# dmalyuta/explicit_hybrid_mpc

Hardware: AMD Instinct MI355X
Metric: oracle LP solves/sec + final regions/sec, 4-state 2-input N=5 hybrid MPC (higher is better)
Workload: dtype f64

## Files before the change

explicit_hybrid_mpc_amd/build.py:

```python

import os
import shutil
import subprocess
from concurrent.futures import ThreadPoolExecutor

HERE = os.path.dirname(os.path.abspath(__file__))
SRC_DIR = os.path.join(HERE, 'csrc')
LIB_DIR = os.path.join(HERE, 'lib')
OBJ_DIR = os.path.join(LIB_DIR, 'obj')
LIB = os.path.join(LIB_DIR, 'libehmpc.so')
def _headers():
    hs = sorted(f for f in os.listdir(SRC_DIR) if f.endswith('.h'))
    return hs + [os.path.join('..', '..', 'include', 'ehmpc.h')]


HEADERS = _headers()
K2_NPS = (8, 12, 16, 20, 24, 28, 32)
K2_SLOTS = (1, 2, 3, 4)
K2Q_NPS = (8, 16, 24, 32)
KP_INSTANCES = tuple((d, e, sl) for (d, e) in ((12, 8), (16, 8), (16, 12), (20, 12), (20, 16),
                                                (24, 16), (24, 20), (28, 20), (28, 24), (32, 24),
                                                (32, 28)) for sl in (2, 3)) + \
    ((16, 12, 4), (28, 20, 4), (32, 24, 4))
KPM_INSTANCES = KP_INSTANCES
K3_RS = (2, 4)
MIDFIRST = '-DEHM_PERSIST_MIDFIRST=1'
FLAGS = ['--offload-arch=gfx950', '-O3', '-std=c++17', '-fPIC', '-Wno-unused-result',
         '-fvisibility=hidden', '-fvisibility-inlines-hidden']
FLAGS += os.environ.get('EHM_BUILD_FLAGS', '').split()
_TAG = os.environ.get('EHM_BUILD_TAG', '')
if _TAG:
    OBJ_DIR = os.path.join(LIB_DIR, 'obj_' + _TAG)
    LIB = os.path.join(LIB_DIR, 'libehmpc_%s.so' % _TAG)


def _hipcc():
    for cand in (os.environ.get('HIPCC'), shutil.which('hipcc'), '/opt/rocm/bin/hipcc'):
        if cand and os.path.exists(cand):
            return cand
    raise RuntimeError('hipcc not found: libehmpc.so cannot be built')


def _cxx():
    for cand in (os.environ.get('CXX'), shutil.which('g++'), shutil.which('c++')):
        if cand and os.path.exists(cand):
            return cand
    return _hipcc()


_INC_CACHE = {}


def _includes(path):
    path = os.path.normpath(path)
    if path in _INC_CACHE:
        return _INC_CACHE[path]
    _INC_CACHE[path] = found = set()
    try:
        text = open(path).read()
    except OSError:
        return found
    import re
    for inc in re.findall(r'^\s*#\s*include\s+"([^"]+)"', text, flags=re.M):
        dep = os.path.normpath(os.path.join(os.path.dirname(path), inc))
        if os.path.exists(dep):
            found.add(dep)
            found |= _includes(dep)
    return found


def _dep_mtime(src=None):
    if src is None:
        deps = [os.path.normpath(os.path.join(SRC_DIR, h)) for h in HEADERS]
    else:
        deps = list(_includes(src))
    deps += [__file__]
    return max(os.path.getmtime(d) for d in deps)


SEARCH_SRC = os.path.join(SRC_DIR, 'ehm_search.cpp')
SEARCH_OBJ = os.path.join(OBJ_DIR, 'ehm_search.o')
FRONTIER_SRC = os.path.join(SRC_DIR, 'ehm_frontier.cpp')
FRONTIER_OBJ = os.path.join(OBJ_DIR, 'ehm_frontier.o')
SEARCH_DEPS = [SEARCH_SRC, os.path.normpath(os.path.join(HERE, '..', 'include', 'ehm_search.h')),
               os.path.normpath(os.path.join(HERE, '..', 'include', 'ehmpc.h'))]
FRONTIER_DEPS = [FRONTIER_SRC,
                 os.path.normpath(os.path.join(HERE, '..', 'include', 'ehm_frontier.h'))] + \
    SEARCH_DEPS[1:]
HOST_OBJECTS = ((SEARCH_OBJ, SEARCH_SRC, SEARCH_DEPS), (FRONTIER_OBJ, FRONTIER_SRC, FRONTIER_DEPS))


def _objects():
    objs = [(os.path.join(OBJ_DIR, 'ehm_capi.o'), os.path.join(SRC_DIR, 'ehm_capi.hip'), []),
            (os.path.join(OBJ_DIR, 'ehm_explicit.o'), os.path.join(SRC_DIR, 'ehm_explicit.hip'),
             []),
            (os.path.join(OBJ_DIR, 'ehm_implicit.o'), os.path.join(SRC_DIR, 'ehm_implicit.hip'),
             [])]
    for np_ in K2_NPS:
        for sl in K2_SLOTS:
            objs.append((os.path.join(OBJ_DIR, 'ehm_k2_%d_%d.o' % (np_, sl)),
                         os.path.join(SRC_DIR, 'ehm_k2.hip'),
                         ['-DEHM_NP=%d' % np_, '-DEHM_SLOTS=%d' % sl, MIDFIRST]))
    for np_ in K2Q_NPS:
        for sl in K2_SLOTS:
            objs.append((os.path.join(OBJ_DIR, 'ehm_k2q_%d_%d.o' % (np_, sl)),
                         os.path.join(SRC_DIR, 'ehm_k2.hip'),
                         ['-DEHM_NP=%d' % np_, '-DEHM_SLOTS=%d' % sl, '-DEHM2_QUAD=1', MIDFIRST]))
    for npd, npe, sl in KP_INSTANCES:
        objs.append((os.path.join(OBJ_DIR, 'ehm_kp_%d_%d_%d.o' % (npd, npe, sl)),
                     os.path.join(SRC_DIR, 'ehm_kp.hip'),
                     ['-DEHM_NPD=%d' % npd, '-DEHM_NPE=%d' % npe, '-DEHM_SLOTS=%d' % sl]))
    for npd, npe, sl in KPM_INSTANCES:
        objs.append((os.path.join(OBJ_DIR, 'ehm_kpm_%d_%d_%d.o' % (npd, npe, sl)),
                     os.path.join(SRC_DIR, 'ehm_kp.hip'),
                     ['-DEHM_NPD=%d' % npd, '-DEHM_NPE=%d' % npe, '-DEHM_SLOTS=%d' % sl,
                      '-DEHM_PERSIST_MIDFIRST=1']))
    for rs in K3_RS:
        objs.append((os.path.join(OBJ_DIR, 'ehm_k3_%d.o' % rs),
                     os.path.join(SRC_DIR, 'ehm_k3.hip'),
                     ['-DEHM3_RS=%d' % rs, '-mllvm', '-pragma-unroll-threshold=200000']))
    objs.append((os.path.join(OBJ_DIR, 'ehm_k4.o'), os.path.join(SRC_DIR, 'ehm_k4.hip'), []))
    return objs


def _stale(obj, src, dep_t):
    return (not os.path.exists(obj) or
            os.path.getmtime(obj) < max(dep_t, os.path.getmtime(src)))


def is_stale():
    if not os.path.exists(LIB):
        return True
    t = os.path.getmtime(LIB)
    srcs = [os.path.join(SRC_DIR, f)
            for f in ('ehm_capi.hip', 'ehm_k2.hip', 'ehm_k3.hip', 'ehm_k4.hip', 'ehm_kp.hip',
                      'ehm_explicit.hip', 'ehm_implicit.hip')]
    return max([_dep_mtime()] + [os.path.getmtime(s)
                                 for s in srcs + SEARCH_DEPS + FRONTIER_DEPS]) > t


def build(force=False, verbose=False, jobs=None):
    if not force and not is_stale():
        return LIB
    os.makedirs(OBJ_DIR, exist_ok=True)
    hipcc = _hipcc()
    todo = [(o, s, f) for (o, s, f) in _objects() if force or _stale(o, s, _dep_mtime(s))]

    def compile_one(item):
        obj, src, extra = item
        cmd = [hipcc] + FLAGS + extra + ['-c', src, '-o', obj]
        if verbose:
            print(' '.join(cmd))
        subprocess.check_call(cmd)

    jobs = jobs or max(1, (os.cpu_count() or 2))
    with ThreadPoolExecutor(max_workers=jobs) as pool:
        list(pool.map(compile_one, todo))
    for obj, src, deps in HOST_OBJECTS:
        if force or not os.path.exists(obj) or \
                os.path.getmtime(obj) < max(os.path.getmtime(d) for d in deps):
            cmd = [_cxx(), '-O2', '-std=c++17', '-fPIC', '-Wall', '-fvisibility=hidden', '-fvisibility-inlines-hidden',
                   '-c', src, '-o', obj]
            if verbose:
                print(' '.join(cmd))
            subprocess.check_call(cmd)
    cmd = [hipcc, '--offload-arch=gfx950', '-shared', '-fPIC'] + [o for (o, _, _) in _objects()]
    cmd += [obj for obj, _, _ in HOST_OBJECTS]
    cmd += ['-o', LIB]
    if verbose:
        print(' '.join(cmd))
    subprocess.check_call(cmd)
    return LIB


if __name__ == '__main__':
    print(build(force=True, verbose=True))
```

explicit_hybrid_mpc_amd/csrc/ehm_ipm2.h:

```cpp
#include "ehm_dev.h"

#ifndef EHM_NP
#error "EHM_NP (column capacity, multiple of 4) must be defined"
#endif
#ifndef EHM_SLOTS
#error "EHM_SLOTS (row slots per lane) must be defined"
#endif

#ifndef EHM2_UNROLL
#define EHM2_UNROLL 2
#endif
#ifndef EHM2_FORM_MFMA
#define EHM2_FORM_MFMA 0
#endif
#ifndef EHM2_LU_CHUNK
#define EHM2_LU_CHUNK 8
#endif
#define EHM2_TOL_RES      1e-10
#define EHM2_TOL_GAP      1e-10
#define EHM2_MAX_ITER     40
#define EHM2_STEP_FRAC    0.999
#define EHM2_STEP_FRAC_SAFE 0.99
#define EHM2_STEP_FRAC_LAST 0.9
#define EHM2_ATTEMPTS     3
#define EHM2_PIVOT_REL    1e-13
#define EHM2_PIVOT_BIG    1e128
#define EHM2_STALL_ZONE   1e4
#define EHM2_ACCEPT_MERIT 1e3

#define EHM2_CAT2(a, b, c) a##b##_##c
#define EHM2_CAT(a, b, c) EHM2_CAT2(a, b, c)
#ifndef EHM2_QUAD
#define EHM2_QUAD 0
#endif
#if EHM2_QUAD
#define EHM2_NS EHM2_CAT(ehm2q_, EHM_NP, EHM_SLOTS)
#else
#define EHM2_NS EHM2_CAT(ehm2_, EHM_NP, EHM_SLOTS)
#endif

#ifndef EHM2_PROF
#define EHM2_PROF 0
#endif

namespace EHM2_NS {

using namespace ehm;

#if EHM2_PROF
#define EHM2_PT(k)                                                                   \
    {                                                                                \
        const long long _t = (long long)__builtin_readcyclecounter();               \
        if (lane0 == 0) W.pf[k] += (unsigned long long)(_t - _tp);                   \
        _tp = _t;                                                                    \
    }
#define EHM2_PDUMP()                                                                 \
    {                                                                                \
        wsync();                                                                     \
        if (S.gprof && lane0 < 24)                                                   \
            atomicAdd(&S.gprof[lane0], W.pf[lane0] + (lane0 == 23 ? 1ULL : 0ULL));   \
    }
#elif defined(EHM2_ISA_MARKS)
#define EHM2_PT(k) asm volatile("; @@PHASE " #k);
#define EHM2_PDUMP()
#else
#define EHM2_PT(k)
#define EHM2_PDUMP()
#endif

constexpr int NP = EHM_NP;
constexpr int SLOTS = EHM_SLOTS;
constexpr int MROWS = 64 * SLOTS;

__device__ __forceinline__ void wsync() {
    __builtin_amdgcn_fence(__ATOMIC_ACQ_REL, "wavefront");
    __builtin_amdgcn_wave_barrier();
}

template <int CTRL, int ROW_MASK>
__device__ __forceinline__ double dpp_move(double identity, double v) {
    const int lo = __builtin_amdgcn_update_dpp(__double2loint(identity), __double2loint(v), CTRL,
                                               ROW_MASK, 0xf, false);
    const int hi = __builtin_amdgcn_update_dpp(__double2hiint(identity), __double2hiint(v), CTRL,
                                               ROW_MASK, 0xf, false);
    return __hiloint2double(hi, lo);
}
__device__ __forceinline__ double lane63(double v) {
    const int lo = __builtin_amdgcn_readlane(__double2loint(v), 63);
    const int hi = __builtin_amdgcn_readlane(__double2hiint(v), 63);
    return __hiloint2double(hi, lo);
}
#define EHM2_DPP_REDUCE(OP, IDENT)                                       \
    v = OP(v, dpp_move<0x111, 0xf>(IDENT, v));                           \
    v = OP(v, dpp_move<0x112, 0xf>(IDENT, v));                           \
    v = OP(v, dpp_move<0x114, 0xf>(IDENT, v));                           \
    v = OP(v, dpp_move<0x118, 0xf>(IDENT, v));                           \
    v = OP(v, dpp_move<0x142, 0xa>(IDENT, v));                           \
    v = OP(v, dpp_move<0x143, 0xc>(IDENT, v));                           \
    return lane63(v);
__device__ __forceinline__ double op_add(double a, double b) { return a + b; }
__device__ __forceinline__ double op_max(double a, double b) { return fmax(a, b); }
__device__ __forceinline__ double op_min(double a, double b) { return fmin(a, b); }
#ifdef EHM2_REDUCE_SHFL
__device__ __forceinline__ double wave_sum(double v) {
    for (int o = 32; o > 0; o >>= 1) v += __shfl_xor(v, o, 64);
    return v;
}
__device__ __forceinline__ double wave_max(double v) {
    for (int o = 32; o > 0; o >>= 1) v = fmax(v, __shfl_xor(v, o, 64));
    return v;
}
#else
__device__ __forceinline__ double wave_sum(double v) { EHM2_DPP_REDUCE(op_add, 0.0) }
__device__ __forceinline__ double wave_max(double v) {
    EHM2_DPP_REDUCE(op_max, -__builtin_huge_val())
}
#endif
__device__ __forceinline__ double readlane_d(double v, int src) {
    const int lo = __builtin_amdgcn_readlane(__double2loint(v), src);
    const int hi = __builtin_amdgcn_readlane(__double2hiint(v), src);
    return __hiloint2double(hi, lo);
}
__device__ __forceinline__ int pin(int x) {
    asm volatile("" : "+v"(x));
    return x;
}
typedef __attribute__((address_space(3))) const volatile double lds_cvdouble;
__device__ __forceinline__ double lds1(const double* p) {
    return *(lds_cvdouble*)p;
}
__device__ __forceinline__ double uniform_d(double v) {
    int lo, hi;
    asm("s_nop 0\n\tv_readfirstlane_b32 %0, %2\n\tv_readfirstlane_b32 %1, %3\n\ts_nop 1"
        : "=s"(lo), "=s"(hi)
        : "v"(__double2loint(v)), "v"(__double2hiint(v)));
    return __hiloint2double(hi, lo);
}
__device__ __forceinline__ double const_d(double literal) {
    int lo = __double2loint(literal), hi = __double2hiint(literal);
    asm volatile("" : "+s"(lo), "+s"(hi));
    return __hiloint2double(hi, lo);
}
__device__ __forceinline__ double frcp(double x) {
    double r = __builtin_amdgcn_rcp(x);
    double e = fma(-x, r, 1.0);
    r = fma(r, e, r);
    e = fma(-x, r, 1.0);
    r = fma(r, e, r);
    return r;
}

struct Shared {
    const double* Wc;
    const double* wv;
    const double* cv;
    const double* aE;
    const double* eval;
    const int* erow;
    const int* eidx;
    int n, m, p, lda;
    int nd0, nE, LE;
    int colS, colOne, colZero;
#if EHM2_PROF
    unsigned long long* gprof;
#endif
};
__host__ __device__ inline size_t shared_doubles(const DevProblem& P) {
    return (((size_t)P.tot4 + (P.wc_lds ? P.m + P.n : 0)) + 1) & ~(size_t)1;
}
__device__ inline void carve_shared(Shared& S, double* base, const DevProblem& P) {
    S.n = P.n; S.m = P.m; S.p = P.p; S.lda = P.lda4;
    S.nd0 = P.nd0; S.nE = P.n - P.nd0; S.LE = P.LE4;
    S.colS = P.nd0; S.colOne = P.nd0 + P.p; S.colZero = P.nd0 + P.p + 1;
#if EHM2_PROF
    S.gprof = nullptr;
#endif
    S.Wc = base;
    S.aE = base + (size_t)(P.nd0 + P.p + 2) * P.lda4;
    S.eval = base + (size_t)P.ncw4 * P.lda4;
    S.erow = reinterpret_cast<const int*>(S.eval + (size_t)S.nE * S.LE);
    S.eidx = S.erow + (size_t)S.nE * S.LE;
    if (P.wc_lds) {
        S.wv = base + P.tot4;
        S.cv = S.wv + P.m;
    } else {
        S.wv = P.w;
        S.cv = P.c;
    }
}
__device__ inline void use_commutation(Shared& S, const DevProblem& P, int d) {
    if (!P.wc_lds) S.wv = P.w + (size_t)d * P.m;
}
__device__ inline void load_shared(const DevProblem& P, int d, double* base, int tid, int nthr) {
    const int tot = P.tot4;
    const double* src = P.Wc4 + (size_t)d * tot;
    for (int k = tid; k < tot; k += nthr) base[k] = src[k];
    if (P.wc_lds) {
        const double* wd = P.w + (size_t)d * P.m;
        for (int k = tid; k < P.m; k += nthr) base[tot + k] = wd[k];
        for (int k = tid; k < P.n; k += nthr) base[tot + P.m + k] = P.c[k];
    }
}

struct Wave {
    double* M;
    double* X;
    double* vm0;
    double* vm1;
    double* c;
    double* x;
    double* xb;
    double* t;
    double* ub;
    double* db;
    double* sc;
    int n_lp, ne, ldx, ldm, xbase;
    int nr;
    int nE;
    int n_lin;
    int spec_col;
    int n_mpc;
    const double* E;
    double* yv;
    int psi0, npsi;
    int nsx;
    double sign_floor;
    double* gE;
    double* iD;
    double* qE;
    double* hX;
    double* xh;
    double* dn;
#if EHM2_PROF
    unsigned long long* pf;
#endif
#if EHM2_QUAD
    double* Q;
    double* qv;
    double* a1;
    double* a2;
    double* gv;
    double* lq;
    int quad;
    int eq;
    double kap0, kap1, kap2, v0, bq1, bq2;
#endif
};
constexpr int LDM = NP + 1;
constexpr int GS = NP + 1;
typedef double double2v __attribute__((ext_vector_type(2)));
typedef double double4v __attribute__((ext_vector_type(4)));

__host__ __device__ constexpr int u_row_start(int k) {
    return (k & 1) ? (k * NP - 2 * (k / 2) * (k / 2)) : (k * NP - 2 * (k / 2) * (k / 2 - 1));
}
__host__ __device__ constexpr int uoff(int k) { return u_row_start(k) - (k & ~1); }
constexpr int U_SIZE = NP * (NP + 2) / 2;
constexpr size_t A_MIN = (size_t)U_SIZE + 256 + MROWS;
constexpr size_t A_KS = 512;
constexpr size_t A_SQ = ((size_t)NP * LDM < A_KS) ? A_KS : (size_t)NP * LDM;
constexpr size_t A_DOUBLES = (A_MIN < A_SQ) ? A_SQ : A_MIN;
__host__ __device__ inline int dense_rows(int ne, int p) { return (ne > p) ? ne - (p + 1) : ne; }
__host__ __device__ inline size_t wave_lp_doubles(int n_lp, int ne, int nE, int p) {
    const int kd = dense_rows(ne, p);
    const size_t ldx = kd ? ((size_t)kd | 1) : 0;
    const size_t nf = ((size_t)n_lp + 1) & ~(size_t)1;
    const size_t nEp = ((size_t)nE + 1) & ~(size_t)1;
    size_t tot = A_DOUBLES + (size_t)n_lp * ldx + 4 * nf + 2 * (size_t)NP + ((size_t)NP + 16) +
                 (size_t)nE * GS + 4 * nEp + 2 * (size_t)NP + 8;
#if EHM2_QUAD
    tot += 5 * (size_t)NP + (size_t)NP * LDM + 2;
#endif
#if EHM2_PROF
    tot += 24;
#endif
    return (tot + 1) & ~(size_t)1;
}
__device__ inline void carve_wave(Wave& W, double* base, int n_lp, int ne, int m, int nE, int nsx) {
    W.n_lp = n_lp;
    W.nE = nE;
    W.nr = n_lp - nE;
    W.ne = ne;
    W.ldm = LDM;
    W.ldx = (ne > nsx) ? ((ne - nsx) | 1) : 0;
    W.xbase = lp_xbase(m, ne);
    if (ne > 0 && W.xbase < 64 * (SLOTS - 1)) W.xbase = 64 * (SLOTS - 1);
    const int nf = (n_lp + 1) & ~1;
    const int nEp = (nE + 1) & ~1;
    W.M = base;
    W.vm0 = base + U_SIZE;
    W.sc = base + U_SIZE;
    W.vm1 = base + U_SIZE + 256;
    base += A_DOUBLES;
    W.X = base;   base += (size_t)n_lp * W.ldx;
    W.c = base;   base += nf;
    W.x = base;   base += nf;
    W.xb = base;  base += nf;
    W.t = base;   base += nf;
    W.ub = base;  base += NP;
    W.db = base;  base += NP;
    W.yv = base;  base += NP + 16;
    W.gE = base;  base += (size_t)nE * GS;
    W.iD = base;  base += nEp;
    W.qE = base;  base += nEp;
    W.hX = base;  base += 2 * nEp;
    W.xh = base;  base += 2 * NP;
    W.dn = base;  base += 8;
#if EHM2_PROF
    W.pf = reinterpret_cast<unsigned long long*>(base);  base += 24;
#endif
#if EHM2_QUAD
    W.qv = base;  base += NP;
    W.a1 = base;  base += NP;
    W.a2 = base;  base += NP;
    W.gv = base;  base += NP;
    W.lq = base;  base += 2;
    W.Q = base;
    W.quad = 0;
    W.eq = -1;
// ... 380 lines not shown
#pragma unroll
            for (int q = 0; q < 4; ++q)
#pragma unroll
                for (int r = 0; r < 4; ++r) acc[q][r] = fma(aj[q], ak[r], acc[q][r]);
        }
    }
    constexpr int EPR = 16 / R;
    if (KS > 1) {
#pragma unroll
        for (int rd = 0; rd < R; ++rd) {
            wsync();
            if (active) {
                double* sc = W.M + (size_t)h * EPR * TA + task;
#pragma unroll
                for (int q = 0; q < 4; ++q)
#pragma unroll
                    for (int r = 0; r < 4; ++r) {
                        const int en = 4 * q + r - rd * EPR;
                        if (en >= 0 && en < EPR) sc[en * TA] = acc[q][r];
                    }
            }
            wsync();
            for (int v = lane; v < EPR * TA; v += 64) {
                double sum = W.M[v];
#pragma unroll
                for (int hh = 1; hh < KS; ++hh) sum += W.M[(size_t)hh * EPR * TA + v];
                W.M[v] = sum;
            }
            wsync();
            if (h == 0) {
#pragma unroll
                for (int q = 0; q < 4; ++q)
#pragma unroll
                    for (int r = 0; r < 4; ++r) {
                        const int en = 4 * q + r - rd * EPR;
                        if (en >= 0 && en < EPR) acc[q][r] = W.M[en * TA + task];
                    }
            }
        }
    }
    wsync();
    if (h == 0) {
#pragma unroll
        for (int q = 0; q < 4; ++q)
#pragma unroll
            for (int r = 0; r < 4; ++r) {
                const int jj = 4 * bj + q, kk = 4 * bk + r;
                W.M[jj * LDM + kk] = acc[q][r];
                W.M[kk * LDM + jj] = acc[q][r];
            }
    }
}

template <int KS>
__device__ __forceinline__ void form_blocks_ks(const Shared& S, const Wave& W, const double* dvec,
                                               int lane, int nbA, int TA) {
    const int tot1 = KS * 16 * TA;
    if (tot1 <= (int)A_KS) form_blocks<KS, 1>(S, W, dvec, lane, nbA, TA);
    else if (tot1 <= 2 * (int)A_KS) form_blocks<KS, 2>(S, W, dvec, lane, nbA, TA);
    else form_blocks<KS, 4>(S, W, dvec, lane, nbA, TA);
}

__device__ __forceinline__ void form_mfma(const Shared& S, const Wave& W, const double* dvec,
                                          int lane, int ncols) {
    const int li = lane & 15, lk = lane >> 4;
    const bool two = (NP > 16) && ncols > 16;
    const double* zero = S.Wc + (size_t)S.colZero * S.lda;
    const int j0 = li, j1 = 16 + li;
    const double* p0 = (j0 < ncols) ? (S.Wc + (size_t)wc_col(W, j0) * S.lda) : zero;
    const double* p1 = (j1 < ncols) ? (S.Wc + (size_t)wc_col(W, j1) * S.lda) : zero;
    double4v c00 = {0.0, 0.0, 0.0, 0.0}, c10 = {0.0, 0.0, 0.0, 0.0}, c11 = {0.0, 0.0, 0.0, 0.0};
    const int m = S.m;
    const int m4 = m & ~3;
    p0 += lk;
    p1 += lk;
    const double* pd = dvec + lk;
    int i0 = 0;
    if (!two) {
        double4v c0b = {0.0, 0.0, 0.0, 0.0};
        for (; i0 + 16 <= m4; i0 += 16) {
            double d[4], w[4];
#pragma unroll
            for (int u = 0; u < 4; ++u) {
                d[u] = lds1(pd + i0 + 4 * u);
                w[u] = lds1(p0 + i0 + 4 * u);
            }
            c00 = __builtin_amdgcn_mfma_f64_16x16x4f64(w[0] * d[0], w[0], c00, 0, 0, 0);
            c0b = __builtin_amdgcn_mfma_f64_16x16x4f64(w[1] * d[1], w[1], c0b, 0, 0, 0);
            c00 = __builtin_amdgcn_mfma_f64_16x16x4f64(w[2] * d[2], w[2], c00, 0, 0, 0);
            c0b = __builtin_amdgcn_mfma_f64_16x16x4f64(w[3] * d[3], w[3], c0b, 0, 0, 0);
        }
#pragma unroll
        for (int r = 0; r < 4; ++r) c00[r] += c0b[r];
    }
    for (; i0 < m4; i0 += 4) {
        const double d = lds1(pd + i0);
        const double w0 = lds1(p0 + i0);
        const double a0 = w0 * d;
        c00 = __builtin_amdgcn_mfma_f64_16x16x4f64(a0, w0, c00, 0, 0, 0);
        if (two) {
            const double w1 = lds1(p1 + i0);
            const double a1 = w1 * d;
            c10 = __builtin_amdgcn_mfma_f64_16x16x4f64(a1, w0, c10, 0, 0, 0);
            c11 = __builtin_amdgcn_mfma_f64_16x16x4f64(a1, w1, c11, 0, 0, 0);
        }
    }
    if (m4 < m) {
        const bool in = m4 + lk < m;
        const int ic = in ? m4 : (m - 1 - lk);
        const double d = in ? lds1(pd + ic) : 0.0;
        const double w0 = lds1(p0 + ic);
        const double a0 = w0 * d;
        c00 = __builtin_amdgcn_mfma_f64_16x16x4f64(a0, w0, c00, 0, 0, 0);
        if (two) {
            const double w1 = lds1(p1 + ic);
            const double a1 = w1 * d;
            c10 = __builtin_amdgcn_mfma_f64_16x16x4f64(a1, w0, c10, 0, 0, 0);
            c11 = __builtin_amdgcn_mfma_f64_16x16x4f64(a1, w1, c11, 0, 0, 0);
        }
    }
    for (int e0 = 0; e0 < W.nE; e0 += 4) {
        const int e = e0 + lk;
        const bool in = e < W.nE;
        const int ec = in ? e : 0;
        const double id = W.iD[ec];
        const double g0 = (in && j0 < NP) ? W.gE[ec * GS + (j0 < NP ? j0 : 0)] : 0.0;
        c00 = __builtin_amdgcn_mfma_f64_16x16x4f64(-g0 * id, g0, c00, 0, 0, 0);
        if (two) {
            const double g1 = (in && j1 < NP) ? W.gE[ec * GS + (j1 < NP ? j1 : 0)] : 0.0;
            c10 = __builtin_amdgcn_mfma_f64_16x16x4f64(-g1 * id, g0, c10, 0, 0, 0);
            c11 = __builtin_amdgcn_mfma_f64_16x16x4f64(-g1 * id, g1, c11, 0, 0, 0);
        }
    }
    wsync();
#pragma unroll
    for (int r = 0; r < 4; ++r) {
        const int row = lk + 4 * r, col = li;
        if (row < NP && col < NP) W.M[row * LDM + col] = c00[r];
        if (two) {
            if (16 + row < NP && col < NP) {
                W.M[(16 + row) * LDM + col] = c10[r];
                W.M[col * LDM + 16 + row] = c10[r];
            }
            if (16 + row < NP && 16 + col < NP) W.M[(16 + row) * LDM + 16 + col] = c11[r];
        }
    }
}

__device__ __forceinline__ void form_eliminated(const Shared& S, const Wave& W, const double* dvec,
                                                int lane) {
    constexpr int NPG = (NP > 16) ? 32 : 16;
    const double* zero = S.Wc + (size_t)S.colZero * S.lda;
    const int ntask = W.nE * NPG;
    for (int t0 = 0; t0 < ntask; t0 += 64) {
        const int t = t0 + lane;
        const int r = t & (NPG - 1);
        const int e = t / NPG;
        const bool in = t < ntask;
        const double* col = (in && r < W.n_mpc) ? (S.Wc + (size_t)wc_col(W, r) * S.lda) : zero;
        const int eb = (in ? e : 0) * S.LE;
        double g = 0.0, dl = 0.0;
        for (int k = 0; k < S.LE; k += 4) {
            int i[4];
            double ev[4], dv[4], av[4];
#pragma unroll
            for (int u = 0; u < 4; ++u) {
                i[u] = S.erow[eb + k + u];
                ev[u] = S.eval[eb + k + u];
            }
#pragma unroll
            for (int u = 0; u < 4; ++u) {
                dv[u] = lds1(dvec + i[u]);
                av[u] = lds1(col + i[u]);
            }
#pragma unroll
            for (int u = 0; u < 4; ++u) {
                const double de = dv[u] * ev[u];
                g = fma(de, av[u], g);
                dl = fma(de, ev[u], dl);
            }
        }
        if (in && r < NP) W.gE[e * GS + r] = g;
        if (in && r == 0) W.iD[e] = frcp(dl);
    }
    wsync();
}

__device__ __forceinline__ double row16_sum(double v) {
    v += dpp_move<0x111, 0xf>(0.0, v);
    v += dpp_move<0x112, 0xf>(0.0, v);
    v += dpp_move<0x114, 0xf>(0.0, v);
    v += dpp_move<0x118, 0xf>(0.0, v);
    return readlane_d(v, 15);
}
__device__ __forceinline__ double few_sum(double v, int cnt) {
    return (cnt <= 16) ? row16_sum(v) : wave_sum(v);
}

template <int P>
__device__ __forceinline__ void to_beta_form(const Wave& W, const double* dext, int lane) {
    const int p0 = W.psi0;
    const double* Em = W.E;
    double tmp[P];
    if (lane < NP) {
        double* mr = W.M + lane * LDM + p0;
        double v[P];
#pragma unroll
        for (int r = 0; r < P; ++r) v[r] = mr[r];
#pragma unroll
        for (int q = 0; q < P; ++q) {
            double a = 0.0;
#pragma unroll
            for (int r = 0; r < P; ++r) a = fma(v[r], Em[r * P + q], a);
            tmp[q] = a;
        }
#pragma unroll
        for (int q = 0; q < P; ++q) mr[q] = tmp[q];
    }
    for (int e = lane; e < W.nE; e += 64) {
        double* gr = W.gE + e * GS + p0;
        double v[P];
#pragma unroll
        for (int r = 0; r < P; ++r) v[r] = gr[r];
#pragma unroll
        for (int q = 0; q < P; ++q) {
            double a = 0.0;
#pragma unroll
            for (int r = 0; r < P; ++r) a = fma(v[r], Em[r * P + q], a);
            gr[q] = a;
        }
    }
    wsync();
    if (lane < NP) {
        double* mc = W.M + p0 * LDM + lane;
        double v[P];
#pragma unroll
        for (int r = 0; r < P; ++r) v[r] = mc[r * LDM];
#pragma unroll
        for (int q = 0; q < P; ++q) {
            double a = 0.0;
#pragma unroll
            for (int r = 0; r < P; ++r) a = fma(Em[r * P + q], v[r], a);
            tmp[q] = a;
        }
#pragma unroll
        for (int q = 0; q < P; ++q) mc[q * LDM] = tmp[q];
    }
    wsync();
    if (lane < P) {
        const double dsum = dext[P];
        double* mr = W.M + (p0 + lane) * LDM + p0;
#pragma unroll
        for (int q = 0; q < P; ++q) mr[q] += dsum + ((q == lane) ? dext[lane] : 0.0);
    }
    wsync();
}

__device__ __forceinline__ void form_normal_matrix(const Shared& S, const Wave& W, const double* dvec,
                                          const double* dext, int lane
#if EHM2_PROF
                                          , int lane0, long long& _tp
#endif
                                          ) {
    if (W.nE > 0) form_eliminated(S, W, dvec, lane);
    EHM2_PT(2)
    int nbA;
    if (EHM2_FORM_MFMA || W.n_mpc <= 16) {
        nbA = (W.n_mpc > 16 || NP <= 16) ? (NP >> 2) : 4;
        form_mfma(S, W, dvec, lane, W.n_mpc);
    } else {
        nbA = (W.n_mpc + 3) >> 2;
        const int TA = nbA * (nbA + 1) / 2;
        const int ks = 64 / TA;
        if (ks >= 8) form_blocks_ks<8>(S, W, dvec, lane, nbA, TA);
        else if (NP >= 16 && ks >= 6) form_blocks_ks<6>(S, W, dvec, lane, nbA, TA);
        else if (NP >= 20 && ks >= 4) form_blocks_ks<4>(S, W, dvec, lane, nbA, TA);
        else if (NP >= 24 && ks == 3) form_blocks_ks<3>(S, W, dvec, lane, nbA, TA);
        else if (NP >= 28 && ks == 2) form_blocks_ks<2>(S, W, dvec, lane, nbA, TA);
        else if (NP >= 32) form_blocks<1, 1>(S, W, dvec, lane, nbA, TA);
    }
    const int c0 = 4 * nbA;
    if (c0 < NP) {
        const int nrest = NP - c0;
        for (int k = lane; k < nrest * LDM; k += 64) W.M[c0 * LDM + k] = 0.0;
        for (int c = lane & 15; c < nrest; c += 16)
            for (int r = lane >> 4; r < c0; r += 4) W.M[r * LDM + c0 + c] = 0.0;
    }
    wsync();
    EHM2_PT(3)
    if (W.npsi > 0) {
        switch (W.npsi) {
            case 1: to_beta_form<1>(W, dext, lane); break;
            case 2: to_beta_form<2>(W, dext, lane); break;
            case 3: to_beta_form<3>(W, dext, lane); break;
            case 4: to_beta_form<4>(W, dext, lane); break;
            case 5: to_beta_form<5>(W, dext, lane); break;
            case 6: to_beta_form<6>(W, dext, lane); break;
            case 7: to_beta_form<7>(W, dext, lane); break;
            default: to_beta_form<8>(W, dext, lane); break;
        }
    }
}

__device__ __forceinline__ void lu_factor(double (&row)[NP], const Wave& W, int lane) {
    double* U = W.M;
#pragma unroll
    for (int k = 0; k < NP; ++k) {
        const int kk = k & ~1;
        if (lane >= kk && lane < NP) U[uoff(k) + lane] = row[k];
        double piv = readlane_d(row[k], k);
        const double orig = W.db[k];
        wsync();
        const bool bad = !(piv > const_d(EHM2_PIVOT_REL) * orig) || !(piv > 0.0);
        piv = bad ? const_d(EHM2_PIVOT_BIG) : piv;
        const double rinv = frcp(piv);
        if (lane == 0) W.db[k] = rinv;
        const double l = row[k] * rinv;
        row[k] = l;
        if (((k + 1) & 1) && k + 1 < NP) {
            const double ukq = U[uoff(k) + k + 1];
            row[k + 1] = fma(-l, ukq, row[k + 1]);
        }
#pragma unroll
        for (int q = (k + 2) & ~1; q < NP; q += 2) {
            const double2v u = *reinterpret_cast<const double2v*>(U + uoff(k) + q);
            row[q] = fma(-l, u.x, row[q]);
            row[q + 1] = fma(-l, u.y, row[q + 1]);
            if (((q - ((k + 2) & ~1)) / 2) % (EHM2_LU_CHUNK / 2) == EHM2_LU_CHUNK / 2 - 1)
                __builtin_amdgcn_sched_barrier(0);
        }
#pragma unroll
        for (int q = k + 1; q < NP; ++q) asm volatile("" : "+v"(row[q]));
    }
    wsync();
}

__device__ __forceinline__ void masked_fnma(double& bv, double a, double s, unsigned long long mask) {
    unsigned long long sv;
    asm volatile("s_and_saveexec_b64 %[sv], %[m]\n\t"
                 "v_fma_f64 %[bv], -%[a], %[s], %[bv]\n\t"
                 "s_mov_b64 exec, %[sv]\n\t"
                 "s_nop 0"
                 : [bv] "+v"(bv), [sv] "=&s"(sv)
                 : [a] "v"(a), [s] "s"(s), [m] "s"(mask)
                 : "scc");
}

__device__ __forceinline__ double lu_solve(const double (&row)[NP], const Wave& W, double rinv,
                                           double rhs, int lane) {
    double bv = rhs;
#pragma unroll
    for (int k = 0; k < NP - 1; ++k) {
        const double yk = readlane_d(bv, k);
        bv = fma(-row[k], yk, bv);
    }
    const int jl = (lane < NP) ? lane : (NP - 1);
    const double* urow = W.M + uoff(jl);
#pragma unroll
    for (int k = NP - 1; k >= 1; --k) {
        const double xk = readlane_d(bv * rinv, k);
        masked_fnma(bv, urow[k], xk, (1ull << k) - 1ull);
    }
    const double x = bv * rinv;
    if (lane < W.nr) W.t[lane] = x;
    wsync();
    return x;
}

__device__ __forceinline__ void dense_prep(const Shared& S, const Wave& W, const double* dext,
                                           int lane) {
    const int kd = W.ne - W.nsx;
    if (kd <= 0) return;
    const int e0 = W.nsx;
    const int nEp = (W.nE + 1) & ~1;
    const bool two = kd > 1;
    double g11 = frcp(dext[e0]);
    double g22 = two ? frcp(dext[e0 + 1]) : 1.0;
    double g12 = 0.0;
    double x0 = 0.0, x1 = 0.0;
    if (lane < W.nr) {
        x0 = W.X[(size_t)lane * W.ldx];
        x1 = two ? W.X[(size_t)lane * W.ldx + 1] : 0.0;
    }
    if (W.nE > 0) {
        const bool el = lane < W.nE;
        const double* xr = W.X + (size_t)(W.nr + (el ? lane : 0)) * W.ldx;
        const double xe0 = el ? xr[0] : 0.0;
        const double xe1 = (el && two) ? xr[1] : 0.0;
        const double id = el ? W.iD[el ? lane : 0] : 0.0;
        const double h0 = xe0 * id, h1 = xe1 * id;
        if (el) {
            W.hX[lane] = h0;
            W.hX[nEp + lane] = h1;
        }
        wsync();
        if (lane < W.nr)
            for (int e = 0; e < W.nE; ++e) {
                const double g = W.gE[e * GS + lane];
                x0 = fma(-W.hX[e], g, x0);
                x1 = fma(-W.hX[nEp + e], g, x1);
            }
        g11 += few_sum(h0 * xe0, W.nE);
        if (two) {
            g12 = few_sum(h0 * xe1, W.nE);
            g22 += few_sum(h1 * xe1, W.nE);
        }
    }
    const double i1 = frcp(g11);
    const double l = g12 * i1;
    const double i2 = two ? frcp(fma(-l, g12, g22)) : 0.0;
    x1 = fma(-l, x0, x1);
    if (lane < NP) {
        W.xh[lane] = x0;
        W.xh[NP + lane] = two ? x1 : 0.0;
    }
    if (lane == 0) {
        W.dn[0] = l;
        W.dn[1] = i1;
        W.dn[2] = i2;
    }
    wsync();
}

__device__ __forceinline__ double solve_full(const double (&row)[NP], const Shared& S,
                                             const Wave& W, double rinv, double rhs, int lane) {
    const int kd = W.ne - W.nsx;
    const bool two = kd > 1;
    const int e = lane - W.nr;
    const bool el = W.nE > 0 && e >= 0 && e < W.nE;
    const int jl = (lane < NP) ? lane : (NP - 1);
    double rho0 = 0.0, rho1 = 0.0;
    double rr = (lane < W.nr) ? rhs : 0.0;
    if (W.nE > 0) {
        if (el) W.qE[e] = rhs * W.iD[e];
        wsync();
        if (lane < W.nr)
            for (int e2 = 0; e2 < W.nE; ++e2) rr = fma(-W.gE[e2 * GS + lane], W.qE[e2], rr);
        if (kd > 0) {
            const bool l2 = lane < W.nE;
            const double* xr = W.X + (size_t)(W.nr + (l2 ? lane : 0)) * W.ldx;
            const double q = l2 ? W.qE[l2 ? lane : 0] : 0.0;
            rho0 = few_sum(l2 ? xr[0] * q : 0.0, W.nE);
            if (two) rho1 = few_sum(l2 ? xr[1] * q : 0.0, W.nE);
        }
    }
    double l = 0.0, i1 = 0.0, i2 = 0.0;
    if (kd > 0) {
        l = W.dn[0];
        i1 = W.dn[1];
        i2 = W.dn[2];
        rho1 = fma(-l, rho0, rho1);
        rr = fma(-W.xh[jl], i1 * rho0, rr);
        rr = fma(-W.xh[NP + jl], i2 * rho1, rr);
    }
    const double xD = lu_solve(row, W, rinv, rr, lane);
    double y0 = 0.0, y1 = 0.0;
    if (kd > 0 && W.nE > 0) {
        const bool lr = lane < W.nr;
        const double v0 = few_sum(lr ? W.xh[jl] * xD : 0.0, W.nr) + rho0;
        const double v1 = two ? (few_sum(lr ? W.xh[NP + jl] * xD : 0.0, W.nr) + rho1) : 0.0;
        y1 = v1 * i2;
        y0 = fma(-l, y1, v0 * i1);
    }
    if (W.nE > 0) {
        double xE = 0.0;
        if (el) {
            double acc = rhs;
            const double* ge = W.gE + e * GS;
            for (int j = 0; j < W.nr; ++j) acc = fma(-ge[j], W.t[j], acc);
            if (kd > 0) {
                const double* xr = W.X + (size_t)(W.nr + e) * W.ldx;
                acc = fma(-xr[0], y0, acc);
                if (two) acc = fma(-xr[1], y1, acc);
            }
            xE = acc * W.iD[e];
            W.t[W.nr + e] = xE;
        }
        wsync();
        return el ? xE : xD;
    }
    return xD;
}

__device__ __forceinline__ IpmResult ipm_solve(const Shared& S, const Wave& W, const double (&b)[SLOTS],
                                      int lane0, int sign_only, double step_frac,
                                      double* gout = nullptr) {
    int lane = lane0;
    const int n = W.n_lp;
    const int m_lp = S.m + W.ne;
    RowMap rm;
    make_rowmap(rm, S, W, lane);
    double s[SLOTS], lam[SLOTS], v[SLOTS];
    double bmax = 0.0;
#pragma unroll
    for (int sl = 0; sl < SLOTS; ++sl) {
        v[sl] = rm.valid[sl] ? b[sl] : 0.0;
        s[sl] = rm.valid[sl] ? fmax(b[sl], 1.0) : 1.0;
        lam[sl] = rm.valid[sl] ? 1.0 : 0.0;
        bmax = fmax(bmax, fabs(v[sl]));
    }
    const double bnorm = uniform_d(1.0 + wave_max(bmax));
    const double cj = (lane < n) ? W.c[lane] : 0.0;
    const double cnorm = uniform_d(1.0 + wave_max(fabs(cj)));
    step_frac = uniform_d(step_frac);
    if (lane < n) {
        W.x[lane] = 0.0;
        W.xb[lane] = 0.0;
    }
#pragma unroll
    for (int sl = 0; sl < SLOTS; ++sl) {
        if (!rm.valid[sl]) {
            W.vm0[lane + 64 * sl] = 0.0;
            W.vm1[lane + 64 * sl] = 0.0;
        }
    }
    wsync();

#if EHM2_PROF
    if (lane0 < 24) W.pf[lane0] = 0ULL;
    wsync();
    long long _tp = (long long)__builtin_readcyclecounter();
#endif
    IpmResult res;
    res.obj = 0.0;
    res.merit = const_d(1e300);
    res.iters = 0;
    res.status = 1;
    int stall = 0;
    int m_op = __builtin_amdgcn_readfirstlane(m_lp);
    asm volatile("" : "+s"(m_op));
    const double inv_m = uniform_d(frcp((double)m_op));

    for (int it = 0; it <= EHM2_MAX_ITER; ++it) {
        lane = pin(lane0);
#if EHM2_QUAD
        double xQx = 0.0, qx = 0.0, gjj = 0.0;
        if (W.quad) {
            const double xj = (lane < n) ? W.x[lane] : 0.0;
            const double qj = (lane < n) ? W.qv[lane] : 0.0;
            double g = 0.0;
            if (lane < n) {
                const double* qrow = W.Q + lane * LDM;
                for (int k = 0; k < n; ++k) g = fma(qrow[k], W.x[k], g);
            }
            xQx = wave_sum(xj * g);
            qx = wave_sum(xj * qj);
            const double gvj = g + qj;
            gjj = (lane < n) ? W.kap0 * gvj : 0.0;
            if (W.eq >= 0) {
                const double a1j = (lane < n) ? W.a1[lane] : 0.0;
                const double a2j = (lane < n) ? W.a2[lane] : 0.0;
                if (lane < n) {
                    W.X[(size_t)lane * W.ldx + W.eq - W.nsx] = fma(W.kap1, gvj, a1j);
                    W.X[(size_t)lane * W.ldx + W.eq - W.nsx + 1] = fma(W.kap2, gvj, a2j);
                }
                const double a1x = wave_sum(a1j * xj);
                const double a2x = wave_sum(a2j * xj);
                const int e = lane + 64 * (SLOTS - 1) - W.xbase;
                const double Vx = fma(0.5, xQx, qx);
                if (rm.last_extra && e == W.eq) v[SLOTS - 1] = W.bq1 - fma(W.kap1, Vx, a1x);
                if (rm.last_extra && e == W.eq + 1) v[SLOTS - 1] = W.bq2 - fma(W.kap2, Vx, a2x);
            }
            wsync();
        }
#endif
        double r_p[SLOTS], rs[SLOTS];
        double rpmax = 0.0, sl_sum = 0.0, vl_sum = 0.0;
#pragma unroll
        for (int sl = 0; sl < SLOTS; ++sl) {
            r_p[sl] = rm.valid[sl] ? (s[sl] - v[sl]) : 0.0;
            rpmax = fmax(rpmax, fabs(r_p[sl]));
            sl_sum = fma(s[sl], lam[sl], sl_sum);
            vl_sum = fma(v[sl], lam[sl], vl_sum);
            rs[sl] = frcp(s[sl]);
        }
#pragma unroll
        for (int sl = 0; sl < SLOTS; ++sl) {
            if (rm.valid[sl]) {
                W.vm0[lane + 64 * sl] = lam[sl];
                W.vm1[lane + 64 * sl] = lam[sl] * rs[sl] * r_p[sl];
            }
        }
        wsync();
        EHM2_PT(0)
        double atl, atdr;
        cols_times<true>(S, W, W.vm0, W.vm1, W.M, lane, atl, atdr);
        EHM2_PT(1)
        const double cjj = (lane < n) ? W.c[lane] : 0.0;
        const double xjj = (lane < n) ? W.x[lane] : 0.0;
#if EHM2_QUAD
        const double r_d = (lane < n) ? (atl + cjj + gjj) *
            (W.quad ? rsqrt(1.0 + W.Q[lane * LDM + lane]) : 1.0) : 0.0;
        const double cn = W.quad ? (1.0 + wave_max(fmax(fabs(cjj), fabs(gjj)))) : cnorm;
        const double emax = wave_max(fmax(rpmax / bnorm, fabs(r_d) / cn));
        const double sl_tot = wave_sum(sl_sum);
        const double mu = sl_tot * inv_m;
        double pobj = wave_sum(cjj * xjj);
        double dobj = -wave_sum(vl_sum + xjj * atl);
        if (W.quad) {
            pobj += W.kap0 * (fma(0.5, xQx, qx) + W.v0);
            dobj = pobj - sl_tot;
        }
        const double e_g = fabs(pobj - dobj) / (1.0 + fabs(pobj));
#else
        const double r_d = (lane < n) ? (atl + cjj) : 0.0;
        const double emax = wave_max(fmax(rpmax / bnorm, fabs(r_d) / cnorm));
        const double mu = wave_sum(sl_sum) * inv_m;
        const double dobj = -wave_sum(vl_sum + xjj * atl);
        const double pobj = wave_sum(cjj * xjj);
        const double e_g = fabs(pobj - dobj) / (1.0 + fabs(pobj));
#endif
        const double merit = fmax(emax / const_d(EHM2_TOL_RES), e_g / const_d(EHM2_TOL_GAP));
        if (!(mu == mu) || !(pobj == pobj) || fabs(pobj) > const_d(1e300)) {
            res.merit = const_d(1e300);
            res.obj = pobj;
            res.status = 1;
            res.iters = it;
            break;
        }
        if (merit < res.merit) {
            res.merit = uniform_d(merit);
            res.obj = uniform_d(pobj);
            stall = 0;
            if (lane < n) W.xb[lane] = W.x[lane];
        } else if (res.merit < const_d(EHM2_STALL_ZONE)) {
            ++stall;
        }
        res.iters = it;
        if (merit <= 1.0) {
            res.status = 0;
            break;
        }
        if (sign_only && emax <= const_d(EHM2_SIGN_RES) && pobj * dobj > 0.0 &&
            (sign_only == 1 || pobj > 0.0)) {
            const double lo = fmin(fabs(pobj), fabs(dobj));
            if (lo >= W.sign_floor && fabs(pobj - dobj) <= const_d(EHM2_SIGN_GAP) * lo &&
                emax * (1.0 + fabs(pobj)) <= const_d(EHM2_SIGN_RES_REL) * lo) {
                res.obj = pobj;
                res.merit = merit;
                res.margin = lo;
                res.status = 0;
                if (lane < n) W.xb[lane] = W.x[lane];
                wsync();
                EHM2_PT(15)
                EHM2_PDUMP()
                return res;
            }
        }
        if (stall >= 3 || it == EHM2_MAX_ITER || !(merit == merit)) break;

        EHM2_PT(15)
        lane = pin(lane0);
#pragma unroll
        for (int sl = 0; sl < SLOTS; ++sl)
            if (rm.valid[sl]) W.vm0[lane + 64 * sl] = lam[sl] * rs[sl];
        wsync();
        if (rm.last_extra || rm.last_sx >= 0)
            W.ub[lane + 64 * (SLOTS - 1) - W.xbase] = lam[SLOTS - 1] * rs[SLOTS - 1];
#if EHM2_QUAD
        if (W.quad && W.eq >= 0 && rm.last_extra) {
            const int e = lane + 64 * (SLOTS - 1) - W.xbase;
            if (e == W.eq) W.lq[0] = lam[SLOTS - 1];
            if (e == W.eq + 1) W.lq[1] = lam[SLOTS - 1];
        }
#endif
        wsync();
#if EHM2_PROF
        form_normal_matrix(S, W, W.vm0, W.ub, lane, lane0, _tp);
#else
        form_normal_matrix(S, W, W.vm0, W.ub, lane);
#endif
        EHM2_PT(4)
        lane = pin(lane0);
        dense_prep(S, W, W.ub, lane);
        EHM2_PT(5)
        lane = pin(lane0);
        double row[NP];
        {
            const int jr = (lane < NP) ? lane : (NP - 1);
            const double* mrow = W.M + jr * LDM;
#pragma unroll
            for (int q = 0; q < NP; ++q) row[q] = mrow[q];
            double dg = mrow[jr];
            for (int r = 0; r < W.ne - W.nsx; ++r) {
                const double* xh = W.xh + r * NP;
                const double xl = xh[jr];
                const double ce = W.dn[1 + r] * xl;
                dg = fma(ce, xl, dg);
#pragma unroll
                for (int q = 0; q < NP; ++q) {
                    row[q] = fma(ce, xh[q], row[q]);
                    if ((q & 3) == 3) __builtin_amdgcn_sched_barrier(0);
                }
            }
#if EHM2_QUAD
            if (W.quad) {
                double wq = W.kap0;
                if (W.eq >= 0) wq = fma(W.kap1, W.lq[0], fma(W.kap2, W.lq[1], wq));
                const int jl = (lane < NP) ? lane : (NP - 1);
                const double* qrow = W.Q + jl * LDM;
                const bool in = jl < W.n_lp;
#pragma unroll
                for (int q = 0; q < NP; ++q)
                    row[q] = fma(wq, (in && q < W.n_lp) ? qrow[q] : 0.0, row[q]);
                dg = fma(wq, in ? qrow[jl] : 0.0, dg);
            }
#endif
            if (lane < NP) W.db[lane] = dg;
        }
        wsync();
        EHM2_PT(6)
        lu_factor(row, W, lane);
#pragma unroll
        for (int k = 0; k < NP; ++k) row[k] = (k < lane) ? row[k] : 0.0;
        EHM2_PT(7)
        const double rinv_l = W.db[(lane < NP) ? lane : (NP - 1)];

        lane = pin(lane0);
#if EHM2_QUAD
        const double rhs_aff = (lane < n) ? (-cjj - gjj - atdr) : 0.0;
#else
        const double rhs_aff = (lane < n) ? (-cjj - atdr) : 0.0;
#endif
        double dxj = solve_full(row, S, W, rinv_l, rhs_aff, lane);
        EHM2_PT(8)
        double adx[SLOTS];
        rows_times(S, W, lane, W.t, adx);
        EHM2_PT(9)
        double ds_a[SLOTS], dl_a[SLOTS];
        double rho_p = 0.0, rho_d = 0.0;
#pragma unroll
        for (int sl = 0; sl < SLOTS; ++sl) {
            ds_a[sl] = rm.valid[sl] ? (-r_p[sl] - adx[sl]) : 0.0;
            dl_a[sl] = rm.valid[sl] ? (-lam[sl] - lam[sl] * rs[sl] * ds_a[sl]) : 0.0;
            rho_p = fmax(rho_p, -ds_a[sl] * rs[sl]);
            rho_d = fmax(rho_d, rm.valid[sl] ? fma(ds_a[sl], rs[sl], 1.0) : 0.0);
        }
        rho_p = wave_max(rho_p);
        rho_d = wave_max(rho_d);
        double ap = (rho_p > 1.0) ? 1.0 / rho_p : 1.0;
        double ad = (rho_d > 1.0) ? 1.0 / rho_d : 1.0;
#if EHM2_QUAD
        if (W.quad) ap = ad = fmin(ap, ad);
#endif
        double mu_aff = 0.0;
#pragma unroll
        for (int sl = 0; sl < SLOTS; ++sl)
            if (rm.valid[sl])
                mu_aff = fma(s[sl] + ap * ds_a[sl], lam[sl] + ad * dl_a[sl], mu_aff);
        mu_aff = wave_sum(mu_aff) * inv_m;
        const double ratio = mu_aff / mu;
        const double sigma = ratio * ratio * ratio;
        const double smu = sigma * mu;

        lane = pin(lane0);
#pragma unroll
        for (int sl = 0; sl < SLOTS; ++sl) {
            if (rm.valid[sl]) W.vm1[lane + 64 * sl] = (ds_a[sl] * dl_a[sl] - smu) * rs[sl];
        }
        wsync();
        double atc, dummy;
        EHM2_PT(10)
        cols_times<false>(S, W, W.vm1, W.vm1, W.sc, lane, atc, dummy);
        EHM2_PT(11)
        const double rhs = (lane < n) ? (rhs_aff + atc) : 0.0;
        dxj = solve_full(row, S, W, rinv_l, rhs, lane);
        EHM2_PT(12)
        rows_times(S, W, lane, W.t, adx);
        EHM2_PT(13)
        double ds[SLOTS], dl[SLOTS];
        rho_p = 0.0;
        rho_d = 0.0;
#pragma unroll
        for (int sl = 0; sl < SLOTS; ++sl) {
            const double corr = rm.valid[sl] ? W.vm1[lane + 64 * sl] : 0.0;
            const double rl = frcp(rm.valid[sl] ? lam[sl] : 1.0);
            ds[sl] = rm.valid[sl] ? (-r_p[sl] - adx[sl]) : 0.0;
            dl[sl] = rm.valid[sl] ? (-lam[sl] - corr - lam[sl] * rs[sl] * ds[sl]) : 0.0;
            rho_p = fmax(rho_p, -ds[sl] * rs[sl]);
            rho_d = fmax(rho_d, -dl[sl] * rl);
        }
        rho_p = wave_max(rho_p);
        rho_d = wave_max(rho_d);
        ap = (rho_p > step_frac) ? step_frac / rho_p : 1.0;
        ad = (rho_d > step_frac) ? step_frac / rho_d : 1.0;
#if EHM2_QUAD
        if (W.quad) ap = ad = fmin(ap, ad);
#endif
        if (lane < n) W.x[lane] = fma(ap, dxj, W.x[lane]);
#pragma unroll
        for (int sl = 0; sl < SLOTS; ++sl) {
            if (rm.valid[sl]) {
                s[sl] = fma(ap, ds[sl], s[sl]);
                lam[sl] = fma(ad, dl[sl], lam[sl]);
                v[sl] = fma(-ap, adx[sl], v[sl]);
            }
        }
        wsync();
        EHM2_PT(14)
    }
    wsync();
    EHM2_PDUMP()
    if (gout) {
        const bool conv = (res.status == 0) && (res.merit <= 1.0);
        for (int q = 0; q < S.p; ++q) {
            const double* col = S.Wc + (size_t)(S.colS + q) * S.lda + lane0;
            double a = 0.0;
#pragma unroll
            for (int sl = 0; sl < SLOTS; ++sl)
                if (lane0 + 64 * sl < S.m) a = fma(col[64 * sl], lam[sl], a);
            a = wave_sum(a);
            if (lane0 == 0) gout[q] = conv ? a : __builtin_nan("");
        }
        wsync();
    }
    if (res.status != 0 && res.merit <= const_d(EHM2_ACCEPT_MERIT)) res.status = 0;
    res.margin = fabs(res.obj);
    return res;
}

}
```

Measured before the change: 9.868 million.

## Carry affine RHS through LU factorization and chunk reduction loops in IPM solve

Splits solve_full into reduce_rhs, lu_forward, lu_backward and expand_solution. For the smaller persistent midfirst kernels (NPD up to 16), the affine right-hand side is reduced before factorization and its forward substitution is folded into lu_factor through a masked FNMA per pivot, so the separate forward sweep is skipped. It also replaces several serial scalar fma loops over nE and nr with chunked loads (fnma_sum) to give the loads more parallelism. This adds readlanes inside the factor loop and raises register pressure.

Result: slower. 9.715 million (-1.6%).

```diff
diff --git a/explicit_hybrid_mpc_amd/build.py b/explicit_hybrid_mpc_amd/build.py
--- a/explicit_hybrid_mpc_amd/build.py
+++ b/explicit_hybrid_mpc_amd/build.py
@@ -25,6 +25,8 @@
 KPM_INSTANCES = KP_INSTANCES
 K3_RS = (2, 4)
 MIDFIRST = '-DEHM_PERSIST_MIDFIRST=1'
+CARRY_RHS = '-DEHM2_CARRY_RHS=1'
+CARRY_RHS_MAX_NPD = 16
 FLAGS = ['--offload-arch=gfx950', '-O3', '-std=c++17', '-fPIC', '-Wno-unused-result',
          '-fvisibility=hidden', '-fvisibility-inlines-hidden']
 FLAGS += os.environ.get('EHM_BUILD_FLAGS', '').split()
@@ -114,7 +116,8 @@
         objs.append((os.path.join(OBJ_DIR, 'ehm_kpm_%d_%d_%d.o' % (npd, npe, sl)),
                      os.path.join(SRC_DIR, 'ehm_kp.hip'),
                      ['-DEHM_NPD=%d' % npd, '-DEHM_NPE=%d' % npe, '-DEHM_SLOTS=%d' % sl,
-                      '-DEHM_PERSIST_MIDFIRST=1']))
+                      '-DEHM_PERSIST_MIDFIRST=1'] +
+                     ([CARRY_RHS] if npd <= CARRY_RHS_MAX_NPD else [])))
     for rs in K3_RS:
         objs.append((os.path.join(OBJ_DIR, 'ehm_k3_%d.o' % rs),
                      os.path.join(SRC_DIR, 'ehm_k3.hip'),
diff --git a/explicit_hybrid_mpc_amd/csrc/ehm_ipm2.h b/explicit_hybrid_mpc_amd/csrc/ehm_ipm2.h
--- a/explicit_hybrid_mpc_amd/csrc/ehm_ipm2.h
+++ b/explicit_hybrid_mpc_amd/csrc/ehm_ipm2.h
@@ -15,6 +15,12 @@
 #endif
 #ifndef EHM2_LU_CHUNK
 #define EHM2_LU_CHUNK 8
+#endif
+#ifndef EHM2_SUM_CHUNK
+#define EHM2_SUM_CHUNK 8
+#endif
+#ifndef EHM2_CARRY_RHS
+#define EHM2_CARRY_RHS 0
 #endif
 #define EHM2_TOL_RES      1e-10
 #define EHM2_TOL_GAP      1e-10
@@ -1001,39 +1007,6 @@
     }
 }
 
-__device__ __forceinline__ void lu_factor(double (&row)[NP], const Wave& W, int lane) {
-    double* U = W.M;
-#pragma unroll
-    for (int k = 0; k < NP; ++k) {
-        const int kk = k & ~1;
-        if (lane >= kk && lane < NP) U[uoff(k) + lane] = row[k];
-        double piv = readlane_d(row[k], k);
-        const double orig = W.db[k];
-        wsync();
-        const bool bad = !(piv > const_d(EHM2_PIVOT_REL) * orig) || !(piv > 0.0);
-        piv = bad ? const_d(EHM2_PIVOT_BIG) : piv;
-        const double rinv = frcp(piv);
-        if (lane == 0) W.db[k] = rinv;
-        const double l = row[k] * rinv;
-        row[k] = l;
-        if (((k + 1) & 1) && k + 1 < NP) {
-            const double ukq = U[uoff(k) + k + 1];
-            row[k + 1] = fma(-l, ukq, row[k + 1]);
-        }
-#pragma unroll
-        for (int q = (k + 2) & ~1; q < NP; q += 2) {
-            const double2v u = *reinterpret_cast<const double2v*>(U + uoff(k) + q);
-            row[q] = fma(-l, u.x, row[q]);
-            row[q + 1] = fma(-l, u.y, row[q + 1]);
-            if (((q - ((k + 2) & ~1)) / 2) % (EHM2_LU_CHUNK / 2) == EHM2_LU_CHUNK / 2 - 1)
-                __builtin_amdgcn_sched_barrier(0);
-        }
-#pragma unroll
-        for (int q = k + 1; q < NP; ++q) asm volatile("" : "+v"(row[q]));
-    }
-    wsync();
-}
-
 __device__ __forceinline__ void masked_fnma(double& bv, double a, double s, unsigned long long mask) {
     unsigned long long sv;
     asm volatile("s_and_saveexec_b64 %[sv], %[m]\n\t"
@@ -1045,14 +1018,51 @@
                  : "scc");
 }
 
-__device__ __forceinline__ double lu_solve(const double (&row)[NP], const Wave& W, double rinv,
-                                           double rhs, int lane) {
+__device__ __forceinline__ void lu_factor(double (&row)[NP], const Wave& W, int lane, double& aug) {
+    double* U = W.M;
+#pragma unroll
+    for (int k = 0; k < NP; ++k) {
+        const int kk = k & ~1;
+        if (lane >= kk && lane < NP) U[uoff(k) + lane] = row[k];
+        double piv = readlane_d(row[k], k);
+        const double yk = (EHM2_CARRY_RHS && k < NP - 1) ? readlane_d(aug, k) : 0.0;
+        const double orig = W.db[k];
+        wsync();
+        const bool bad = !(piv > const_d(EHM2_PIVOT_REL) * orig) || !(piv > 0.0);
+        piv = bad ? const_d(EHM2_PIVOT_BIG) : piv;
+        const double rinv = frcp(piv);
+        if (lane == 0) W.db[k] = rinv;
+        const double l = row[k] * rinv;
+        row[k] = l;
+        if (EHM2_CARRY_RHS && k < NP - 1) masked_fnma(aug, l, yk, ~((2ull << k) - 1ull));
+        if (((k + 1) & 1) && k + 1 < NP) {
+            const double ukq = U[uoff(k) + k + 1];
+            row[k + 1] = fma(-l, ukq, row[k + 1]);
+        }
+#pragma unroll
+        for (int q = (k + 2) & ~1; q < NP; q += 2) {
+            const double2v u = *reinterpret_cast<const double2v*>(U + uoff(k) + q);
+            row[q] = fma(-l, u.x, row[q]);
+            row[q + 1] = fma(-l, u.y, row[q + 1]);
+            if (((q - ((k + 2) & ~1)) / 2) % (EHM2_LU_CHUNK / 2) == EHM2_LU_CHUNK / 2 - 1)
+                __builtin_amdgcn_sched_barrier(0);
+        }
+#pragma unroll
+        for (int q = k + 1; q < NP; ++q) asm volatile("" : "+v"(row[q]));
+    }
+    wsync();
+}
+
+__device__ __forceinline__ double lu_forward(const double (&row)[NP], double rhs) {
     double bv = rhs;
 #pragma unroll
     for (int k = 0; k < NP - 1; ++k) {
         const double yk = readlane_d(bv, k);
         bv = fma(-row[k], yk, bv);
     }
+    return bv;
+}
+__device__ __forceinline__ double lu_backward(const Wave& W, double rinv, double bv, int lane) {
     const int jl = (lane < NP) ? lane : (NP - 1);
     const double* urow = W.M + uoff(jl);
 #pragma unroll
@@ -1064,6 +1074,23 @@
     if (lane < W.nr) W.t[lane] = x;
     wsync();
     return x;
+}
+
+__device__ __forceinline__ double fnma_sum(const double* a, int sa, const double* b, int sb,
+                                           int n, double acc) {
+    for (int j = 0; j < n; j += EHM2_SUM_CHUNK) {
+        double av[EHM2_SUM_CHUNK], bw[EHM2_SUM_CHUNK];
+#pragma unroll
+        for (int u = 0; u < EHM2_SUM_CHUNK; ++u) {
+            const int ju = (j + u < n) ? (j + u) : (n - 1);
+            av[u] = a[ju * sa];
+            bw[u] = b[ju * sb];
+        }
+#pragma unroll
+        for (int u = 0; u < EHM2_SUM_CHUNK; ++u)
+            if (j + u < n) acc = fma(-av[u], bw[u], acc);
+    }
+    return acc;
 }
 
 __device__ __forceinline__ void dense_prep(const Shared& S, const Wave& W, const double* dext,
@@ -1093,12 +1120,10 @@
             W.hX[nEp + lane] = h1;
         }
         wsync();
-        if (lane < W.nr)
-            for (int e = 0; e < W.nE; ++e) {
-                const double g = W.gE[e * GS + lane];
-                x0 = fma(-W.hX[e], g, x0);
-                x1 = fma(-W.hX[nEp + e], g, x1);
-            }
+        if (lane < W.nr) {
+            x0 = fnma_sum(W.hX, 1, W.gE + lane, GS, W.nE, x0);
+            if (two) x1 = fnma_sum(W.hX + nEp, 1, W.gE + lane, GS, W.nE, x1);
+        }
         g11 += few_sum(h0 * xe0, W.nE);
         if (two) {
             g12 = few_sum(h0 * xe1, W.nE);
@@ -1121,20 +1146,20 @@
     wsync();
 }
 
-__device__ __forceinline__ double solve_full(const double (&row)[NP], const Shared& S,
-                                             const Wave& W, double rinv, double rhs, int lane) {
+__device__ __forceinline__ double reduce_rhs(const Shared& S, const Wave& W, double rhs, int lane,
+                                             double& rho0, double& rho1) {
     const int kd = W.ne - W.nsx;
     const bool two = kd > 1;
     const int e = lane - W.nr;
     const bool el = W.nE > 0 && e >= 0 && e < W.nE;
     const int jl = (lane < NP) ? lane : (NP - 1);
-    double rho0 = 0.0, rho1 = 0.0;
+    rho0 = 0.0;
+    rho1 = 0.0;
     double rr = (lane < W.nr) ? rhs : 0.0;
     if (W.nE > 0) {
         if (el) W.qE[e] = rhs * W.iD[e];
         wsync();
-        if (lane < W.nr)
-            for (int e2 = 0; e2 < W.nE; ++e2) rr = fma(-W.gE[e2 * GS + lane], W.qE[e2], rr);
+        if (lane < W.nr) rr = fnma_sum(W.gE + lane, GS, W.qE, 1, W.nE, rr);
         if (kd > 0) {
             const bool l2 = lane < W.nE;
             const double* xr = W.X + (size_t)(W.nr + (l2 ? lane : 0)) * W.ldx;
@@ -1143,18 +1168,24 @@
             if (two) rho1 = few_sum(l2 ? xr[1] * q : 0.0, W.nE);
         }
     }
-    double l = 0.0, i1 = 0.0, i2 = 0.0;
     if (kd > 0) {
-        l = W.dn[0];
-        i1 = W.dn[1];
-        i2 = W.dn[2];
+        const double l = W.dn[0], i1 = W.dn[1], i2 = W.dn[2];
         rho1 = fma(-l, rho0, rho1);
         rr = fma(-W.xh[jl], i1 * rho0, rr);
         rr = fma(-W.xh[NP + jl], i2 * rho1, rr);
     }
-    const double xD = lu_solve(row, W, rinv, rr, lane);
+    return rr;
+}
+__device__ __forceinline__ double expand_solution(const Shared& S, const Wave& W, double rhs,
+                                                  double xD, double rho0, double rho1, int lane) {
+    const int kd = W.ne - W.nsx;
+    const bool two = kd > 1;
+    const int e = lane - W.nr;
+    const bool el = W.nE > 0 && e >= 0 && e < W.nE;
+    const int jl = (lane < NP) ? lane : (NP - 1);
     double y0 = 0.0, y1 = 0.0;
     if (kd > 0 && W.nE > 0) {
+        const double l = W.dn[0], i1 = W.dn[1], i2 = W.dn[2];
         const bool lr = lane < W.nr;
         const double v0 = few_sum(lr ? W.xh[jl] * xD : 0.0, W.nr) + rho0;
         const double v1 = two ? (few_sum(lr ? W.xh[NP + jl] * xD : 0.0, W.nr) + rho1) : 0.0;
@@ -1164,9 +1195,7 @@
     if (W.nE > 0) {
         double xE = 0.0;
         if (el) {
-            double acc = rhs;
-            const double* ge = W.gE + e * GS;
-            for (int j = 0; j < W.nr; ++j) acc = fma(-ge[j], W.t[j], acc);
+            double acc = fnma_sum(W.gE + e * GS, 1, W.t, 1, W.nr, rhs);
             if (kd > 0) {
                 const double* xr = W.X + (size_t)(W.nr + e) * W.ldx;
                 acc = fma(-xr[0], y0, acc);
@@ -1373,6 +1402,17 @@
         lane = pin(lane0);
         dense_prep(S, W, W.ub, lane);
         EHM2_PT(5)
+        double rho0, rho1, yr = 0.0;
+#if EHM2_CARRY_RHS
+        lane = pin(lane0);
+#if EHM2_QUAD
+        const double rhs_aff = (lane < n) ? (-cjj - gjj - atdr) : 0.0;
+#else
+        const double rhs_aff = (lane < n) ? (-cjj - atdr) : 0.0;
+#endif
+        yr = reduce_rhs(S, W, rhs_aff, lane, rho0, rho1);
+        EHM2_PT(16)
+#endif
         lane = pin(lane0);
         double row[NP];
         {
@@ -1409,19 +1449,26 @@
         }
         wsync();
         EHM2_PT(6)
-        lu_factor(row, W, lane);
+        lu_factor(row, W, lane, yr);
 #pragma unroll
         for (int k = 0; k < NP; ++k) row[k] = (k < lane) ? row[k] : 0.0;
         EHM2_PT(7)
         const double rinv_l = W.db[(lane < NP) ? lane : (NP - 1)];
 
         lane = pin(lane0);
+#if !EHM2_CARRY_RHS
 #if EHM2_QUAD
         const double rhs_aff = (lane < n) ? (-cjj - gjj - atdr) : 0.0;
 #else
         const double rhs_aff = (lane < n) ? (-cjj - atdr) : 0.0;
 #endif
-        double dxj = solve_full(row, S, W, rinv_l, rhs_aff, lane);
+        yr = reduce_rhs(S, W, rhs_aff, lane, rho0, rho1);
+        EHM2_PT(16)
+        yr = lu_forward(row, yr);
+#endif
+        double dxj = lu_backward(W, rinv_l, yr, lane);
+        EHM2_PT(17)
+        dxj = expand_solution(S, W, rhs_aff, dxj, rho0, rho1, lane);
         EHM2_PT(8)
         double adx[SLOTS];
         rows_times(S, W, lane, W.t, adx);
@@ -1463,7 +1510,13 @@
         cols_times<false>(S, W, W.vm1, W.vm1, W.sc, lane, atc, dummy);
         EHM2_PT(11)
         const double rhs = (lane < n) ? (rhs_aff + atc) : 0.0;
-        dxj = solve_full(row, S, W, rinv_l, rhs, lane);
+        yr = reduce_rhs(S, W, rhs, lane, rho0, rho1);
+        EHM2_PT(18)
+        yr = lu_forward(row, yr);
+        EHM2_PT(19)
+        dxj = lu_backward(W, rinv_l, yr, lane);
+        EHM2_PT(20)
+        dxj = expand_solution(S, W, rhs, dxj, rho0, rho1, lane);
         EHM2_PT(12)
         rows_times(S, W, lane, W.t, adx);
         EHM2_PT(13)
```
